# ZhiHuangHn/vtkCloudPoint

Hardware: AMD Instinct MI355X
Metric: Mpoints/s DBSCAN+label @10M pts (higher is better)
Workload: dtype f64; 1 GPU; C4: 10000000-pt cloud (half uniform background, 200 Gaussian blobs), one monolithic DBImproved.dbscan, metric L1_2D, eps 0.1, minPts 10; mode=single, points_total=10000000, points_per_gpu=10000000, clusters=27380, resident_in_hbm=True

## Files before the change

vtkcloudpoint_amd/csrc/dbscan.hip:

```cpp
#include <string.h>

#include <cmath>
#include <cstdlib>
#include <cstring>
#include <limits>
#include <vector>

#include "bounds.hpp"
#include "dbscan_engine.hpp"
#include "grid_common.hpp"

using namespace vcpg;

namespace {

#ifndef VCP_UNR2
#define VCP_UNR2 4
#endif
#ifndef VCP_UNR3
#define VCP_UNR3 2
#endif
#ifndef VCP_UNRW
#define VCP_UNRW 4
#endif
// ... 613 lines not shown
                                                   WorkList wlE, const float* __restrict__ sorted32, Screen sc) {
  const uint32_t p = wl_fetch(wlE);
  if (p == NONE) return;
  float qf[3];
  int cc[3];
  load_pt32<GD>(sorted32, p, qf);
  cell_of32<GD>(qf, g, cc);
  constexpr int UNR = GD == 3 ? VCP_UNR3 : VCP_UNR2;
  const int32_t myg = GROUPED ? sgroup[p] : 0;
  const uint32_t me = (uint32_t)p;
  uint32_t first = me;
  for_rows<GD>(cc, g, ct, [&](uint32_t s, uint32_t e) {
    if (s >= me) return true;
    if (e > me) e = me;
    for (uint32_t j0 = s; j0 < e; j0 += UNR) {
      float rr[UNR][3];
      bool cand[UNR];
#pragma unroll
      for (int u = 0; u < UNR; u++) {
        const uint32_t jj = min(j0 + u, e - 1);
        cand[u] = (j0 + u < e) && (flags[jj] & F_EXPAND);
        if (GROUPED) cand[u] = cand[u] && sgroup[jj] == myg;
        load_pt32<GD>(sorted32, jj, rr[u]);
      }
#pragma unroll
      for (int u = 0; u < UNR; u++)
        if (first == me && cand[u] && within_scr<GD, METRIC>(qf, rr[u], sc, xs, me, j0 + u, thr)) first = j0 + u;
      if (first != me) return false;
    }
    return true;
  });
  if (first != me) parent[me] = first;
}

__global__ __launch_bounds__(TPB) void k_union_init_list(const uint8_t* __restrict__ flags, uint32_t* __restrict__ parent,
                                                        NbrOut no, WorkList wlE) {
  const uint32_t p = wl_fetch(wlE);
  if (p == NONE) return;
  const int nrec = flags[p] >> 4;
  const uint32_t* li = nbr_list(no, p);
  for (int k = 0; k < nrec; k++) {
    const uint32_t j = li[k];
    if (j < p && (flags[j] & F_EXPAND)) {
      parent[p] = j;
      return;
    }
  }
}

template <int JOIN>
__global__ __launch_bounds__(TPB) void k_flatten0(uint32_t* __restrict__ parent, WorkList wlE,
                                                 const uint8_t* __restrict__ flags, NbrOut no) {
  const uint32_t p = wl_fetch(wlE);
  if (p == NONE) return;
  uint32_t r = (uint32_t)p, x = ld_parent_cached(parent, r);
  if (x == r || JOIN == 2) {
    if (!JOIN) return;
    uint32_t rp = JOIN == 2 ? uf_root(parent, p) : p;
    const int nrec = flags[p] >> 4;
    const uint32_t* li = nbr_list(no, p);
    uint32_t s0 = NONE, s1 = NONE, s2 = NONE;
    for (int k = 0; k < nrec; k++) {
      const uint32_t j = li[k];
      if (!(flags[j] & F_EXPAND)) continue;
      const uint32_t y = ld_parent_cached(parent, j);
      if (y == rp || y == s0 || y == s1 || y == s2) continue;
      const uint32_t ry = uf_root(parent, y);
      const uint32_t rm = uf_root(parent, rp);
      s2 = s1;
      s1 = s0;
      s0 = rp;
      rp = (ry != rm) ? uf_link(parent, rm, ry) : rm;
      if (y != rp) s1 = y;
    }
    return;
  }
  while (x != r) {
    r = x;
    x = ld_parent_cached(parent, r);
  }
  __hip_atomic_store(&parent[p], r, __ATOMIC_RELAXED, __HIP_MEMORY_SCOPE_WAVEFRONT);
}

constexpr uint32_t CHUNK_MIXED = 0xFFFFFFFEu;
constexpr int DENSE_PER_CELL = 16;
__global__ __launch_bounds__(TPB) void k_chunkroot(const uint32_t* __restrict__ parent, CellTab ct,
                                                  uint32_t* __restrict__ chunkroot) {
  const uint32_t nin = *ct.nin;
  const int64_t p = (int64_t)blockIdx.x * TPB + threadIdx.x;
  const uint32_t x = p < nin ? parent[p] : NONE;
  const unsigned long long have = __ballot(x != NONE);
  uint32_t out = NONE;
  if (have) {
    const uint32_t r = (uint32_t)__shfl((int)x, __ffsll((long long)have) - 1, 64);
    out = __ballot(x != NONE && x != r) ? CHUNK_MIXED : r;
  }
  if ((threadIdx.x & 63) == 0) chunkroot[p >> 6] = out;
}

#define VCP_JOIN(x)                                                \
  do {                                                             \
    const uint32_t rx__ = uf_root(parent, (x));                    \
    const uint32_t rm__ = uf_root(parent, rp);                     \
    rp = (rx__ != rm__) ? uf_link(parent, rm__, rx__) : rm__;      \
  } while (0)
#define VCP_FLUSH()                                                \
  do {                                                             \
    if (q0 != NONE) {                                              \
      const uint32_t old__ = rp;                                   \
      VCP_JOIN(q0);                                                \
      a2 = a0;                                                     \
      a0 = q0;                                                     \
      a1 = old__;                                                  \
    }                                                              \
    if (q1 != NONE) {                                              \
      VCP_JOIN(q1);                                                \
      a2 = q1;                                                     \
    }                                                              \
    q0 = q1 = NONE;                                                \
  } while (0)

template <int GD, int METRIC, bool GROUPED, bool PRE, bool DENSE = false>
__global__ __launch_bounds__(TPB) void k_union(ExactSrc xs, GridP g, double thr,
                                              CellTab ct,
                                              const int32_t* __restrict__ sgroup, uint32_t* __restrict__ parent,
                                              WorkList wlE, const float* __restrict__ sorted32, Screen sc,
                                              const uint32_t* __restrict__ chunkroot = nullptr) {
  const uint32_t p = wl_fetch(wlE);
  if (p == NONE) return;
  constexpr int NR = GD == 3 ? 9 : 3;
  uint32_t rs[NR], re[NR];
  float qf[3];
  int cc[3];
  load_pt32<GD>(sorted32, p, qf);
  cell_of32<GD>(qf, g, cc);
  row_bounds<GD>(cc, g, ct, rs, re);
  constexpr int UNR = PRE ? VCP_UNRW : (GD == 3 ? VCP_UNR3 : VCP_UNR2);
  const int32_t myg = GROUPED ? sgroup[p] : 0;
  const uint32_t me = (uint32_t)p;
  uint32_t rp = parent[me];
  uint32_t q0 = NONE, q1 = NONE, a0 = NONE, a1 = NONE, a2 = NONE;
#pragma unroll
  for (int r = 0; r < NR; r++) {
    const uint32_t s = rs[r];
    const uint32_t e = min(re[r], me);
    uint32_t last_c = NONE;
    for (uint32_t j0 = s; j0 < e; j0 += UNR) {
      if (DENSE) {
        const uint32_t cj = j0 >> 6;
        if (cj != last_c) {
          last_c = cj;
          if ((cj << 6) >= s && ((cj + 1u) << 6) <= e) {
            const uint32_t cr = chunkroot[cj];
            if (cr == NONE || cr == rp) {
              j0 = ((cj + 1u) << 6) - UNR;
              continue;
            }
          }
        }
      }
      uint32_t pj[UNR];
      float cf[UNR][3];
#pragma unroll
      for (int u = 0; u < UNR; u++) {
        const uint32_t jj = min(j0 + u, e - 1);
        pj[u] = ld_parent_cached(parent, jj);
        if (!PRE) load_pt32<GD>(sorted32, jj, cf[u]);
      }
#pragma unroll
      for (int u = 0; u < UNR; u++) {
        const uint32_t j = j0 + u, x = pj[u];
        if (j >= e || x == NONE || x == rp) continue;
        if (PRE && (x == a0 || x == a1 || x == a2 || x == q0 || x == q1)) continue;
        if (GROUPED && sgroup[j] != myg) continue;
        if (PRE) load_pt32<GD>(sorted32, j, cf[u]);
        if (!within_scr<GD, METRIC>(qf, cf[u], sc, xs, me, j, thr)) continue;
        if (!PRE) {
          const uint32_t x2 = ld_parent_cached(parent, x);
          if (x2 != rp) {
            const uint32_t rx = uf_root(parent, x2);
            const uint32_t rm = uf_root(parent, rp);
            rp = (rx != rm) ? uf_link(parent, rm, rx) : rm;
          }
          if (x != rp && j != rp) __hip_atomic_store(&parent[j], rp, __ATOMIC_RELAXED, __HIP_MEMORY_SCOPE_WAVEFRONT);
        } else if (q0 == NONE) {
          q0 = x;
        } else if (q1 == NONE) {
          q1 = x;
        } else {
          VCP_FLUSH();
          q0 = x;
        }
      }
    }
  }
  VCP_FLUSH();
  if (rp != me) __hip_atomic_store(&parent[me], rp, __ATOMIC_RELAXED, __HIP_MEMORY_SCOPE_AGENT);
}
#undef VCP_FLUSH
#undef VCP_JOIN

template <bool FILTER>
__global__ __launch_bounds__(TPB) void k_flatten(uint32_t* __restrict__ parent, const uint32_t* __restrict__ sord,
                                                uint32_t* __restrict__ minord, WorkList wlE) {
  const uint32_t p = wl_fetch(wlE);
  uint32_t r = NONE, v = NONE;
  if (p != NONE) {
    r = (uint32_t)p;
    uint32_t x = parent[r];
    while (x != r) {
      r = x;
      x = parent[r];
    }
    parent[p] = r;
    v = sord[p];
  }
  unsigned long long todo = __ballot(r != NONE);
  const int lane = threadIdx.x & 63;
  while (todo) {
    int leader = __ffsll((long long)todo) - 1;
    uint32_t lr = __shfl(r, leader, 64);
    bool mine = (r == lr);
    uint32_t m = mine ? v : NONE;
#pragma unroll
    for (int d = 32; d > 0; d >>= 1) m = min(m, (uint32_t)__shfl_xor((int)m, d, 64));
    if (lane == leader &&
        (!FILTER || m < __hip_atomic_load(&minord[lr], __ATOMIC_RELAXED, __HIP_MEMORY_SCOPE_AGENT)))
      atomicMin(&minord[lr], m);
    todo &= ~__ballot(mine);
  }
}

__device__ __forceinline__ uint32_t seed_rank(const uint32_t* __restrict__ bits, const uint32_t* __restrict__ pref,
                                              uint32_t m) {
  const uint32_t w = m >> 5;
  return pref[w] + (uint32_t)__popc(bits[w] & ((1u << (m & 31u)) - 1u));
}
__global__ __launch_bounds__(TPB) void k_seed_popc(const uint32_t* __restrict__ bits, uint32_t nw, uint32_t* __restrict__ cnt) {
  uint32_t w = blockIdx.x * TPB + threadIdx.x;
  if (w < nw) cnt[w] = (uint32_t)__popc(bits[w]);
}

__global__ __launch_bounds__(TPB) void k_seedflag(const uint32_t* __restrict__ parent, const uint32_t* __restrict__ minord,
                                                 uint32_t* __restrict__ seedflag, WorkList wlE) {
  const uint32_t p = wl_fetch(wlE);
  if (p == NONE) return;
  if (parent[p] == p) {
    const uint32_t m = minord[p];
    atomicOr(&seedflag[m >> 5], 1u << (m & 31u));
  }
}

__global__ __launch_bounds__(TPB) void k_rootk(const uint32_t* __restrict__ parent, const uint32_t* __restrict__ minord,
                                              const uint32_t* __restrict__ seedbits, const uint32_t* __restrict__ seedpref,
                                              uint32_t* __restrict__ rootk, uint32_t* __restrict__ clseed, WorkList wlE) {
  const uint32_t p = wl_fetch(wlE);
  if (p == NONE) return;
  if (parent[p] == p) {
    uint32_t k = seed_rank(seedbits, seedpref, minord[p]);
    rootk[p] = k;
    clseed[k] = minord[p];
  }
}

__device__ __forceinline__ void twice_add(unsigned twice, unsigned long long* __restrict__ counters) {
  __shared__ unsigned tw[TPB / 64];
  const unsigned long long m2 = __ballot(twice);
  if ((threadIdx.x & 63) == 0) tw[threadIdx.x >> 6] = (unsigned)__popcll(m2);
  __syncthreads();
  if (threadIdx.x == 0) {
    unsigned t = 0;
    for (int k = 0; k < TPB / 64; k++) t += tw[k];
    if (t) atomicAdd(&counters[CNT_TWICE + (blockIdx.x & (CNT_SPREAD - 1))], (unsigned long long)t);
  }
}

template <int GD, int METRIC, bool GROUPED>
__global__ __launch_bounds__(TPB) void k_border(ExactSrc xs, GridP g, double thr,
                                               CellTab ct,
                                               const int32_t* __restrict__ sgroup, const uint8_t* __restrict__ flags,
                                               const uint32_t* __restrict__ parent, const uint32_t* __restrict__ sord,
                                               const uint32_t* __restrict__ rootk, const uint32_t* __restrict__ clseed,
                                               uint32_t* __restrict__ labk, unsigned long long* __restrict__ counters,
                                               uint32_t* __restrict__ group_twice, WorkList wlB, uint32_t own_lo,
                                               uint32_t own_span, const float* __restrict__ sorted32, Screen sc) {
  const uint32_t p = wl_fetch(wlB);
  unsigned twice = 0;
  if (p != NONE) {
    const uint8_t fl = flags[p];
    uint32_t out = 0;
    {
      float qf[3];
      int cc[3];
      load_pt32<GD>(sorted32, p, qf);
      cell_of32<GD>(qf, g, cc);
      constexpr int UNR = VCP_UNRW;
      const int32_t myg = GROUPED ? sgroup[p] : 0;
      uint32_t mx = 0, mnk = NONE;
      for_rows<GD>(cc, g, ct, [&](uint32_t s, uint32_t e) {
        for (uint32_t j0 = s; j0 < e; j0 += UNR) {
          uint32_t rk[UNR];
#pragma unroll
          for (int u = 0; u < UNR; u++) rk[u] = rootk[min(j0 + u, e - 1)];
#pragma unroll
          for (int u = 0; u < UNR; u++) {
            const uint32_t j = j0 + u, x = rk[u];
            if (j >= e || x == NONE || (x >= mnk && x < mx)) continue;
            if (GROUPED && sgroup[j] != myg) continue;
            float rr[3];
            load_pt32<GD>(sorted32, j, rr);
            if (within_scr<GD, METRIC>(qf, rr, sc, xs, p, j, thr)) {
              mx = max(mx, x + 1u);
              mnk = min(mnk, x);
            }
          }
        }
        return true;
      });
      out = mx;
      if (mx != 0 && !(fl & F_CLASSED) && sord[p] - own_lo < own_span && sord[p] < clseed[mnk]) {
        twice = 1;
        if (GROUPED) atomicAdd(&group_twice[myg], 1u);
      }
    }
    labk[p] = (out << 2) | ((fl & F_CORE) ? 1u : 0u) | ((fl & F_CLASSED) ? 2u : 0u);
  }
  if (!GROUPED) twice_add(twice, counters);
}

template <bool GROUPED>
__global__ __launch_bounds__(TPB) void k_border_list(const int32_t* __restrict__ sgroup, const uint8_t* __restrict__ flags,
                                                    const uint32_t* __restrict__ sord, const uint32_t* __restrict__ rootk,
                                                    const uint32_t* __restrict__ clseed, uint32_t* __restrict__ labk,
                                                    unsigned long long* __restrict__ counters,
                                                    uint32_t* __restrict__ group_twice, NbrOut no, WorkList wlB) {
  const uint32_t p = wl_fetch(wlB);
  unsigned twice = 0;
  if (p != NONE) {
    const uint8_t fl = flags[p];
    const int nrec = fl >> 4;
    uint32_t mx = 0, mnk = NONE;
    const uint32_t* li = nbr_list(no, p);
    for (int k = 0; k < nrec; k++) {
      const uint32_t x = rootk[li[k]];
      if (x == NONE) continue;
// ... 213 lines not shown
  int64_t p = (int64_t)blockIdx.x * TPB + threadIdx.x;
  if (p >= nin) return;
  if ((flags[p] & F_EXPAND) && parent[p] == (uint32_t)p) {
    const uint32_t key = minord[p];
    uint32_t lo = 0, hi = nmap;
    while (lo < hi) {
      const uint32_t mid = (lo + hi) >> 1;
      if (map_rep[mid] < key) lo = mid + 1; else hi = mid;
    }
    if (lo < nmap && map_rep[lo] == key) {
      rootk[p] = map_k[lo];
    } else {
      rootk[p] = 0;
      atomicAdd(missing, 1ull);
    }
  }
}

__global__ __launch_bounds__(TPB) void k_slab_output(int64_t n, const uint32_t* __restrict__ pos,
                                                    const uint32_t* __restrict__ labk, const int32_t* __restrict__ tab_gid,
                                                    int32_t* __restrict__ labels, uint8_t* __restrict__ is_classed) {
  int64_t i = (int64_t)blockIdx.x * TPB + threadIdx.x;
  if (i >= n) return;
  const uint32_t k1 = labk[pos[i]] >> 2;
  const int32_t lab = k1 ? tab_gid[k1 - 1] : 0;
  labels[i] = lab;
  if (is_classed) is_classed[i] = lab != 0;
}

double l2_threshold(double eps) {
  if (std::isinf(eps)) return eps;
  double t = eps * eps;
  if (std::isinf(t)) t = std::numeric_limits<double>::max();
  while (std::sqrt(t) > eps) t = std::nextafter(t, 0.0);
  for (;;) {
    double u = std::nextafter(t, std::numeric_limits<double>::infinity());
    if (std::isinf(u) || std::sqrt(u) > eps) break;
    t = u;
  }
  return t;
}

Screen screen_bounds(int metric, int gd, double thr, double E) {
  Screen sc;
  sc.lo = -1.0f;
  sc.hi = INFINITY;
  if (!(thr >= 0.0) || !std::isfinite(E)) return sc;
  if ((thr > 0.0 && thr < 1e-30) || E > 1e18) return sc;
  const double u = 5.9604644775390625e-08;
  const double alpha = 2.0 * u * E * (1.0 + 2.0 * u);
  double err;
  bool lo_ok = true;
  if (metric == VCP_L1_2D) {
    err = 2.0 * alpha * (1.0 + u) + 2.0 * u * (1.0 + u) * thr;
  } else {
    err = 2.0 * alpha * std::sqrt((double)gd * thr) * (1.0 + u) + (double)gd * alpha * alpha + 6.0 * u * (1.0 + u) * thr;
    lo_ok = std::sqrt(thr) > 4.0 * alpha * std::sqrt((double)gd);
  }
  err = err * 1.0625 + 1e-14 * thr + 1e-300;
  const double lo = thr - err, hi = thr + err;
  if (std::isfinite(hi)) {
    float h = (float)hi;
    if ((double)h < hi) h = std::nextafterf(h, INFINITY);
    sc.hi = h;
  }
  if (lo_ok && lo >= 0.0 && std::isfinite(lo)) {
    float l = (float)lo;
    if ((double)l > lo) l = std::nextafterf(l, -INFINITY);
    sc.lo = l;
  } else if (lo_ok && std::isinf(thr) && thr > 0) {
    sc.lo = 3.4028234663852886e38f;
  }
  return sc;
}

unsigned list_perblk(int64_t n) {
  const int64_t band = (n + 8 * LCHUNK - 1) / (8 * LCHUNK) + 1;
  return vcp_blocks(band, TPB);
}

struct Switches {
  int64_t cells_per_point;
  bool screen_off, lists_off, core_global;
  int core_cap, join_all;
};
const Switches& switches() {
  static const Switches sw = [] {
    Switches s;
    const char* e = getenv("VCP_CELL_BUDGET");
    const long v = e ? atol(e) : 32;
    s.cells_per_point = (int64_t)(v < 1 ? 1 : v > 4096 ? 4096 : v);
    s.screen_off = getenv("VCP_NO_SCREEN") != nullptr;
    s.lists_off = getenv("VCP_NO_LISTS") != nullptr;
    s.core_global = getenv("VCP_CORE_GLOBAL") != nullptr;
    s.core_cap = getenv("VCP_CORE_CAP") ? atoi(getenv("VCP_CORE_CAP")) : -1;
    s.join_all = getenv("VCP_JOIN_ALL") ? atoi(getenv("VCP_JOIN_ALL")) : -1;
    return s;
  }();
  return sw;
}

struct EnginePinned {
  double bounds[8];
  uint32_t unclassed;
  uint32_t n_comp;
  unsigned long long counters[CNT_WORDS];
};
static_assert(sizeof(EnginePinned) <= 1024, "the engine's region of vcp_ctx::pinned");
EnginePinned* engine_pinned(vcp_ctx* ctx) { return reinterpret_cast<EnginePinned*>(ctx->pinned); }

struct Call {
  const double* d_coords;
  int64_t n;
  int stride, metric;
  double eps;
  int min_pts;
  int32_t cf_in;
  const uint8_t* d_in_classed;
  int32_t* d_labels;
  uint8_t *d_is_core, *d_is_classed;
  int32_t* cf_out;
  int64_t* dist_evals;
  const DbscanExt* ext;
  int gd = 2;
  unsigned nb = 0;
  const int32_t* d_group = nullptr;
  const uint32_t* d_ord = nullptr;
  uint32_t* d_group_twice = nullptr;
  int G = 0, glo = 0, ghi = 0;
  bool slab = false;
  double* h = nullptr;
  bool all_finite = false;
  double thr = 0.0;
  GridP g;
  Screen sc{-1.0f, INFINITY};
  bool flags_set = false, part_out = false;
  ExactSrc xs{nullptr, nullptr, 0};
  NbrOut no{nullptr, nullptr, 0, 0};
};
void call_derive(Call& c) {
  const DbscanExt* ext = c.ext;
  const bool grouped = ext && ext->d_group;
  c.gd = c.metric == VCP_L2_3D ? 3 : 2;
  c.nb = vcp_blocks(c.n, TPB);
  c.d_group = grouped ? ext->d_group : nullptr;
  c.d_ord = ext ? ext->d_ord : nullptr;
  c.d_group_twice = grouped ? ext->d_group_twice : nullptr;
  c.G = grouped ? ext->G : 0;
  c.glo = grouped ? ext->only_lo : 0;
  c.ghi = grouped ? (ext->only_hi < 0 ? c.G : ext->only_hi) : 0;
  c.slab = ext && ext->slab;
}
BoundsSrc bounds_src(const Call& c) { return BoundsSrc{c.d_coords, c.n, c.gd, c.stride, c.d_group, c.glo, c.ghi}; }

struct MiscView {
  double* d_part;
  double* d_bounds;
  unsigned long long* counters;
  uint32_t* d_total;
};
struct Workspace : MiscView {
  uint4* ctwords;
  uint32_t* ctdense;
  uint32_t* ctcount;
  CellTab ct;
  uint32_t *cellof, *pos, *sord, *parent, *minord, *rootk, *clseed, *labk;
  float* sorted32;
  uint8_t* flags;
  int32_t* sgroup;
  uint32_t nw;
  uint32_t* seedflag;
  uint32_t* seedpref;
  uint32_t *blkE, *blkB;
  WorkList wlE, wlB;
  unsigned nbl;
};

int ws_reserve_misc(vcp_ctx* ctx, int64_t n) {
  return vcp_ensure(ctx, ctx->b_misc, (size_t)(vcp_bounds_parts(n) * 8 + 96) * sizeof(double));
}
MiscView misc_carve(vcp_ctx* ctx, int64_t n) {
  MiscView m;
  m.d_part = ctx->b_misc.as<double>();
  m.d_bounds = m.d_part + (size_t)vcp_bounds_parts(n) * 8;
  m.counters = reinterpret_cast<unsigned long long*>(m.d_bounds + 8);
  m.d_total = reinterpret_cast<uint32_t*>(m.counters + CNT_SEED_TOTAL);
  return m;
}
static_assert((8 + CNT_WORDS) <= 96, "b_misc: bounds and counters behind the partials");

int ws_reserve(vcp_ctx* ctx, int64_t n, unsigned nb, int gd, bool grouped, uint32_t ncells) {
  const size_t ctw = vcp_ct_words(ncells), ctd = vcp_ct_dense_cap(n, ncells);
  VCP_TRY(vcp_ensure(ctx, ctx->b_ctw, ctw * 16 + 64));
  VCP_TRY(vcp_ensure(ctx, ctx->b_ctd, ctd * 128));
  VCP_TRY(vcp_ensure(ctx, ctx->b_cellof, (size_t)n * 4));
  VCP_TRY(vcp_ensure(ctx, ctx->b_pos, (size_t)n * 4));
  VCP_TRY(vcp_ensure(ctx, ctx->b_sorted32, (size_t)n * (gd == 2 ? 2 : 4) * 4));
  VCP_TRY(vcp_ensure(ctx, ctx->b_sidx, (size_t)n * 4));
  VCP_TRY(vcp_ensure(ctx, ctx->b_flags, (size_t)n));
  VCP_TRY(vcp_ensure(ctx, ctx->b_parent, (size_t)n * 4));
  VCP_TRY(vcp_ensure(ctx, ctx->b_minord, (size_t)n * 4));
  const uint32_t nw = (uint32_t)(n / 32 + 2);
  VCP_TRY(vcp_ensure(ctx, ctx->b_seedflag, ((size_t)nw * 2 + 8) * 4));
  VCP_TRY(vcp_ensure(ctx, ctx->b_rootcl, (size_t)n * 4));
  VCP_TRY(vcp_ensure(ctx, ctx->b_clseed, (size_t)n * 4));
  VCP_TRY(vcp_ensure(ctx, ctx->b_labk, (size_t)n * 4));
  if (grouped) VCP_TRY(vcp_ensure(ctx, ctx->b_sgroup, (size_t)n * 4));
  VCP_TRY(vcp_ensure(ctx, ctx->b_wl, ((size_t)n * 2 + (size_t)(nb + 2) * 2) * 4 + 256));
  return VCP_OK;
}
Workspace ws_carve(vcp_ctx* ctx, int64_t n, unsigned nb, bool grouped, uint32_t ncells) {
  Workspace w;
  static_cast<MiscView&>(w) = misc_carve(ctx, n);
  w.ctwords = ctx->b_ctw.as<uint4>();
  w.ctdense = ctx->b_ctd.as<uint32_t>();
  w.ctcount = reinterpret_cast<uint32_t*>(ctx->b_ctw.as<char>() + vcp_ct_words(ncells) * 16);
  w.ct = CellTab{w.ctwords, w.ctdense, w.ctcount + 1};
  w.cellof = ctx->b_cellof.as<uint32_t>();
  w.pos = ctx->b_pos.as<uint32_t>();
  w.sorted32 = ctx->b_sorted32.as<float>();
  w.sord = ctx->b_sidx.as<uint32_t>();
  w.flags = ctx->b_flags.as<uint8_t>();
  w.parent = ctx->b_parent.as<uint32_t>();
  w.minord = ctx->b_minord.as<uint32_t>();
  w.nw = (uint32_t)(n / 32 + 2);
  w.seedflag = ctx->b_seedflag.as<uint32_t>();
  w.seedpref = w.seedflag + ((w.nw + 3) & ~3u);
  w.rootk = ctx->b_rootcl.as<uint32_t>();
  w.clseed = ctx->b_clseed.as<uint32_t>();
  w.labk = ctx->b_labk.as<uint32_t>();
  w.sgroup = grouped ? ctx->b_sgroup.as<int32_t>() : nullptr;
  w.blkE = ctx->b_wl.as<uint32_t>();
  w.blkB = w.blkE + (nb + 2);
  w.wlE.list = w.blkB + (nb + 2);
  w.wlB.list = w.wlE.list + n;
  w.wlE.scan = w.blkE;
  w.wlB.scan = w.blkB;
  w.wlE.nblk = w.wlB.nblk = nb;
  w.wlE.perblk = w.wlB.perblk = list_perblk(n);
  w.nbl = 8u * LCHUNK * w.wlE.perblk;
  return w;
}

struct Totals {
  uint32_t K;
  unsigned long long unclassed;
  unsigned long long twice;
  unsigned long long slot0;
  unsigned long long group_evals;
};
int read_totals(vcp_ctx* ctx, const MiscView& ws, Totals& t) {
  unsigned long long* hc = engine_pinned(ctx)->counters;
  VCP_HIP(ctx, hipMemcpyAsync(hc, ws.counters, CNT_WORDS * sizeof(unsigned long long), hipMemcpyDeviceToHost, ctx->stream));
  VCP_TRY(vcp_phase_finish(ctx));
  VCP_HIP(ctx, hipStreamSynchronize(ctx->stream));
  t.K = *reinterpret_cast<uint32_t*>(hc + CNT_SEED_TOTAL);
  t.slot0 = hc[CNT_LONELY];
  t.group_evals = hc[CNT_GROUP_EVALS];
  t.unclassed = t.twice = 0;
  for (int k = 0; k < CNT_SPREAD; k++) {
    t.unclassed += hc[CNT_UNCLASSED + k];
    t.twice += hc[CNT_TWICE + k];
  }
  return VCP_OK;
}

int stage_bounds(vcp_ctx* ctx, Call& c) {
  vcp_phase(ctx, "bounds");
  VCP_TRY(ws_reserve_misc(ctx, c.n));
  double* h = engine_pinned(ctx)->bounds;
  if (c.ext && c.ext->h_bbox) {
    for (int a = 0; a < 6; a++) h[a] = c.ext->h_bbox[a];
    h[6] = 0.0;
  } else {
    const MiscView m = misc_carve(ctx, c.n);
    VCP_TRY(vcp_bounds(ctx, bounds_src(c), m.d_part, m.d_bounds, h));
  }
  c.h = h;
  c.all_finite = h[6] == 0.0;
  return VCP_OK;
}

int unclassed_ranks(vcp_ctx* ctx, const Call& c, uint32_t* f, uint32_t* d_total) {
  VCP_LAUNCH(ctx, k_unclassed_flag, dim3(c.nb), dim3(TPB), 0, ctx->stream, c.d_in_classed, f, c.n);
  return vcp_exclusive_scan_u32(ctx, f, f, c.n, d_total);
}

template <int GD, int METRIC>
double box_measure(const double* h) {
  const double wx = h[3] - h[0], wy = h[4] - h[1], wz = GD == 3 ? h[5] - h[2] : 0.0;
  return METRIC == VCP_L1_2D ? std::fabs(wx) + std::fabs(wy)
         : METRIC == VCP_L2_2D ? wx * wx + wy * wy : wx * wx + wy * wy + wz * wz;
}

int run_all_pairs(vcp_ctx* ctx, const Call& c) {
  hipStream_t st = ctx->stream;
  const int64_t n = c.n;
  vcp_phase(ctx, "all_pairs");
  VCP_TRY(vcp_ensure(ctx, ctx->b_seedflag, (size_t)(n + 2) * 4));
  uint32_t* f = ctx->b_seedflag.as<uint32_t>();
  uint32_t* d_tot = reinterpret_cast<uint32_t*>(misc_carve(ctx, n).counters);
  unsigned long long unclassed = (unsigned long long)n;
  if (c.d_in_classed) {
    VCP_TRY(unclassed_ranks(ctx, c, f, d_tot));
    uint32_t* hu = &engine_pinned(ctx)->unclassed;
    VCP_HIP(ctx, hipMemcpyAsync(hu, d_tot, 4, hipMemcpyDeviceToHost, st));
    VCP_HIP(ctx, hipStreamSynchronize(st));
    unclassed = hu[0];
  }
  const int core = n >= (int64_t)c.min_pts;
  const int have_seed = unclassed > 0;
  VCP_LAUNCH(ctx, k_all_pairs, dim3(c.nb), dim3(TPB), 0, st, c.d_in_classed, n, core, have_seed, c.cf_in, c.d_labels,
                  c.d_is_core, c.d_is_classed);
  VCP_TRY(vcp_phase_finish(ctx));
  VCP_HIP(ctx, hipStreamSynchronize(st));
  const int made = core && have_seed;
  if (c.cf_out) *c.cf_out = c.cf_in + made;
  if (c.dist_evals) *c.dist_evals = (int64_t)(unclassed + (unsigned long long)made) * n;
  return VCP_OK;
}

int grid_geometry(vcp_ctx* ctx, Call& c, const Switches& sw, double& Emax) {
  const int GD = c.gd;
// ... 58 lines not shown
      if (d > 1048576) d = 1048576;
      g.D[a] = (int)d;
      ncells *= d;
    }
    if (ncells <= budget || std::isinf(cellw)) break;
    cellw *= 1.25;
  }
  if (ncells > budget) return vcp_fail(ctx, VCP_ERR_TOO_LARGE, "grid does not fit the cell budget");
  Emax = 0.0;
  for (int a = 0; a < GD; a++) Emax = std::fmax(Emax, std::fmax(std::fabs(bbox[a] - g.mn[a]), std::fabs(bbox[3 + a] - g.mn[a])));
  if (!std::isfinite(Emax))
    return vcp_fail(ctx, VCP_ERR_UNSUPPORTED, "the cloud's extent overflows binary64 (coordinate - origin is infinite)");
  g.scale = 1.0;
  if (Emax > 1e30 || (Emax > 0.0 && Emax < 1e-20)) g.scale = std::ldexp(1.0, -std::ilogb(Emax));
  g.inv_h = std::isinf(cellw) ? 0.0 : 1.0 / (cellw * g.scale);
  g.ncells = (uint32_t)ncells;
  return VCP_OK;
}

int stage_grid_build(vcp_ctx* ctx, Call& c, const Workspace& ws) {
  GridBuildArgs ga;
  ga.d_coords = c.d_coords;
  ga.n = c.n;
  ga.stride = c.stride;
  ga.gd = c.gd;
  ga.g = c.g;
  ga.d_group = c.d_group;
  ga.glo = c.glo;
  ga.ghi = c.ghi;
  ga.d_ord = c.d_ord;
  ga.d_in_classed = c.d_in_classed;
  ga.ctwords = ws.ctwords;
  ga.ctdense = ws.ctdense;
  ga.ctcount = ws.ctcount;
  ga.sidx = c.d_ord ? ws.cellof : nullptr;
  ga.sorted32 = ws.sorted32;
  ga.sord = ws.sord;
  ga.sgroup = ws.sgroup;
  ga.flags = ws.flags;
  ga.pos = c.part_out ? nullptr : ws.pos;
  VCP_TRY(vcp_grid_build_partition(ctx, ga));
  c.xs = ExactSrc{c.d_coords, c.d_ord ? ws.cellof : ws.sord, c.stride};
  return VCP_OK;
}

template <int GD, int METRIC, bool GROUPED>
int stage_core(vcp_ctx* ctx, Call& c, const Workspace& ws, const Switches& sw) {
  hipStream_t st = ctx->stream;
  const int64_t n = c.n;
  const unsigned nb = c.nb;
  vcp_phase(ctx, "core_count");
  NbrOut& no = c.no;
  if (!sw.lists_off && !c.d_in_classed && !c.slab && c.min_pts >= 2 && c.min_pts <= 16) {
    no.NB = c.min_pts - 1;
    VCP_TRY(vcp_ensure(ctx, ctx->b_nbr, (size_t)no.NB * (size_t)nb * TPB * 4));
    VCP_TRY(vcp_ensure(ctx, ctx->b_nboff, (size_t)nb * TPB * 2));
    no.nbr = ctx->b_nbr.as<uint32_t>();
    no.off = ctx->b_nboff.as<uint16_t>();
    no.core_cap = (GD == 2 && (uint64_t)n < (uint64_t)c.g.ncells) ? std::min(no.NB, CORE_LIST) : no.NB;
    if (sw.core_cap >= 0) no.core_cap = std::min(no.NB, sw.core_cap);
  }
  const size_t lds_nb = (size_t)no.NB * TPB * 4;
  bool tiled = false;
  if constexpr (GD == 2) {
    if (!GROUPED || !sw.core_global) {
      VCP_LAUNCH(ctx, (k_core_lds<GD, METRIC, GROUPED>), dim3(nb), dim3(TPB), 0, st, c.xs, c.g, c.thr, c.min_pts, ws.ct,
                      ws.sgroup, ws.flags, ws.parent, ws.minord, ws.blkE, ws.blkB, no, ws.sorted32, c.sc, c.flags_set);
      tiled = true;
    }
  }
  if (!tiled)
    VCP_LAUNCH(ctx, (k_core<GD, METRIC, GROUPED>), dim3(nb), dim3(TPB), 2 * lds_nb, st, c.xs, c.g, c.thr, c.min_pts, ws.ct,
                    ws.sgroup, ws.flags, ws.parent, ws.minord, ws.blkE, ws.blkB, no, ws.sorted32, c.sc, c.flags_set);
  VCP_TRY(vcp_exclusive_scan_u32(ctx, ws.blkE, ws.blkE, 2 * ((int64_t)nb + 2), nullptr));
  VCP_LAUNCH(ctx, k_wl_fill, dim3(nb), dim3(TPB), 0, st, ws.flags, ws.ct, ws.blkE, ws.blkB, ws.wlE.list, ws.wlB.list,
                  ws.seedflag, ws.nw, ws.counters, c.d_group_twice, (uint32_t)(GROUPED ? c.G : 0));
  return VCP_OK;
}

template <int GD, int METRIC, bool GROUPED>
int stage_union(vcp_ctx* ctx, const Call& c, const Workspace& ws, const Switches& sw) {
  hipStream_t st = ctx->stream;
  const int64_t n = c.n;
  const unsigned nb = c.nb, nbl = ws.nbl;
  const GridP& g = c.g;
  const NbrOut& no = c.no;
  vcp_phase(ctx, "union");
  const bool pre = GD == 2 || no.NB > 0;
  if (no.NB > 0) {
    VCP_LAUNCH(ctx, k_union_init_list, dim3(nbl), dim3(TPB), 0, st, ws.flags, ws.parent, no, ws.wlE);
    const bool all = sw.join_all >= 0 ? sw.join_all != 0 : (uint64_t)n >= (uint64_t)g.ncells;
    if (all) VCP_LAUNCH(ctx, k_flatten0<2>, dim3(nbl), dim3(TPB), 0, st, ws.parent, ws.wlE, ws.flags, no);
    else VCP_LAUNCH(ctx, k_flatten0<1>, dim3(nbl), dim3(TPB), 0, st, ws.parent, ws.wlE, ws.flags, no);
    VCP_LAUNCH(ctx, k_flatten0<0>, dim3(nbl), dim3(TPB), 0, st, ws.parent, ws.wlE, ws.flags, no);
  } else if (GD == 2) {
    VCP_LAUNCH(ctx, (k_union_init<GD, METRIC, GROUPED>), dim3(nbl), dim3(TPB), 0, st, c.xs, g, c.thr, ws.ct, ws.sgroup,
                    ws.flags, ws.parent, ws.wlE, ws.sorted32, c.sc);
    VCP_LAUNCH(ctx, k_flatten0<0>, dim3(nbl), dim3(TPB), 0, st, ws.parent, ws.wlE, ws.flags, no);
  }
  const bool dense = pre && (uint64_t)n > (uint64_t)DENSE_PER_CELL * g.ncells;
  if (dense) {
    VCP_TRY(vcp_ensure(ctx, ctx->b_aux0, ((size_t)nb * (TPB / 64) + 2) * 4));
    uint32_t* chunkroot = ctx->b_aux0.as<uint32_t>();
    VCP_LAUNCH(ctx, k_chunkroot, dim3(nb), dim3(TPB), 0, st, ws.parent, ws.ct, chunkroot);
    VCP_LAUNCH(ctx, (k_union<GD, METRIC, GROUPED, true, true>), dim3(nbl), dim3(TPB), 0, st, c.xs, g, c.thr, ws.ct,
                    ws.sgroup, ws.parent, ws.wlE, ws.sorted32, c.sc, chunkroot);
  } else if (pre)
    VCP_LAUNCH(ctx, (k_union<GD, METRIC, GROUPED, true>), dim3(nbl), dim3(TPB), 0, st, c.xs, g, c.thr, ws.ct, ws.sgroup,
                    ws.parent, ws.wlE, ws.sorted32, c.sc);
  else
    VCP_LAUNCH(ctx, (k_union<GD, METRIC, GROUPED, false>), dim3(nbl), dim3(TPB), 0, st, c.xs, g, c.thr, ws.ct, ws.sgroup,
                    ws.parent, ws.wlE, ws.sorted32, c.sc);
  return VCP_OK;
}

int stage_slab_handoff(vcp_ctx* ctx, const Call& c, const Workspace& ws) {
  hipStream_t st = ctx->stream;
  const unsigned nb = c.nb;
  vcp_phase(ctx, "slab_components");
  VCP_LAUNCH(ctx, k_slab_count, dim3(nb), dim3(TPB), 0, st, ws.parent, ws.flags, ws.ct, ws.blkE);
  VCP_TRY(vcp_exclusive_scan_u32(ctx, ws.blkE, ws.blkE, (int64_t)nb + 1, nullptr));
  VCP_LAUNCH(ctx, k_slab_fill, dim3(nb), dim3(TPB), 0, st, ws.parent, ws.flags, ws.minord, ws.ct, ws.blkE, ws.clseed);
  VCP_LAUNCH(ctx, k_slab_out, dim3(nb), dim3(TPB), 0, st, c.n, ws.pos, ws.flags, ws.parent, ws.minord, c.ext->d_slab_rep,
                  c.d_is_core);
  uint32_t* hn = &engine_pinned(ctx)->n_comp;
  VCP_HIP(ctx, hipMemcpyAsync(hn, ws.blkE + nb, 4, hipMemcpyDeviceToHost, st));
  VCP_TRY(vcp_phase_finish(ctx));
  VCP_HIP(ctx, hipStreamSynchronize(st));
  if (!ctx->slab) ctx->slab = new SlabState();
  SlabState& ss = *ctx->slab;
  ss.valid = true;
  ss.gd = c.gd;
  ss.metric = c.metric;
  ss.n = c.n;
  ss.n_comp = hn[0];
  ss.g = c.g;
  ss.thr = c.thr;
  ss.sc = c.sc;
  ss.xs = c.xs;
  ss.nb = nb;
  if (c.cf_out) *c.cf_out = (int32_t)hn[0];
  return VCP_OK;
}

template <bool GROUPED>
int stage_flatten_number(vcp_ctx* ctx, const Call& c, const Workspace& ws) {
  hipStream_t st = ctx->stream;
  const unsigned nbl = ws.nbl;
  vcp_phase(ctx, "flatten_number");
  if ((uint64_t)c.n >= (uint64_t)c.g.ncells)
    VCP_LAUNCH(ctx, k_flatten<true>, dim3(nbl), dim3(TPB), 0, st, ws.parent, ws.sord, ws.minord, ws.wlE);
  else
    VCP_LAUNCH(ctx, k_flatten<false>, dim3(nbl), dim3(TPB), 0, st, ws.parent, ws.sord, ws.minord, ws.wlE);
  if (!GROUPED && c.slab) return stage_slab_handoff(ctx, c, ws);
  VCP_LAUNCH(ctx, k_seedflag, dim3(nbl), dim3(TPB), 0, st, ws.parent, ws.minord, ws.seedflag, ws.wlE);
  VCP_LAUNCH(ctx, k_seed_popc, dim3(vcp_blocks(ws.nw, TPB)), dim3(TPB), 0, st, ws.seedflag, ws.nw, ws.seedpref);
  VCP_TRY(vcp_exclusive_scan_u32(ctx, ws.seedpref, ws.seedpref, ws.nw, ws.d_total));
  VCP_LAUNCH(ctx, k_rootk, dim3(nbl), dim3(TPB), 0, st, ws.parent, ws.minord, ws.seedflag, ws.seedpref, ws.rootk, ws.clseed,
                  ws.wlE);
  return VCP_OK;
}

template <int GD, int METRIC, bool GROUPED>
int stage_border(vcp_ctx* ctx, const Call& c, const Workspace& ws) {
  hipStream_t st = ctx->stream;
  vcp_phase(ctx, "border");
  VCP_LAUNCH(ctx, k_labk_rest, dim3(c.nb), dim3(TPB), 0, st, ws.flags, ws.parent, ws.rootk, ws.labk, ws.ct);
  if (c.no.NB > 0)
    VCP_LAUNCH(ctx, k_border_list<GROUPED>, dim3(ws.nbl), dim3(TPB), 0, st, ws.sgroup, ws.flags, ws.sord, ws.rootk,
                    ws.clseed, ws.labk, ws.counters, c.d_group_twice, c.no, ws.wlB);
  else
    VCP_LAUNCH(ctx, (k_border<GD, METRIC, GROUPED>), dim3(ws.nbl), dim3(TPB), 0, st, c.xs, c.g, c.thr, ws.ct, ws.sgroup,
                    ws.flags, ws.parent, ws.sord, ws.rootk, ws.clseed, ws.labk, ws.counters, c.d_group_twice, ws.wlB, 0u,
                    NONE, ws.sorted32, c.sc);
  return VCP_OK;
}

template <int GD, bool GROUPED>
int stage_output(vcp_ctx* ctx, const Call& c, const Workspace& ws) {
  hipStream_t st = ctx->stream;
  const int64_t n = c.n;
  const unsigned nb = c.nb;
  const DbscanExt* ext = c.ext;
  if (c.part_out) {
    GridOutputArgs oa;
    oa.n = n;
    oa.sord = ws.sord;
    oa.labk = ws.labk;
    oa.have_in_classed = c.d_in_classed != nullptr;
    oa.cf_in = c.cf_in;
    oa.labels = c.d_labels;
    oa.is_core = c.d_is_core;
    oa.is_classed = c.d_is_classed;
    oa.counters = ws.counters;
    VCP_TRY(vcp_grid_output_partition(ctx, oa));
  } else {
    vcp_phase(ctx, "output");
    VCP_LAUNCH(ctx, (k_output<GROUPED>), dim3(nb), dim3(TPB), 0, st, n, ws.pos, ws.labk, c.d_in_classed, c.d_group,
                    GROUPED ? ext->d_groupstart : nullptr, ws.seedflag, ws.seedpref, c.cf_in, c.d_labels, c.d_is_core,
                    c.d_is_classed, ws.counters);
  }
  if (!GROUPED && c.min_pts <= 0 && !c.all_finite)
    VCP_LAUNCH(ctx, k_lonely_seeds<GD>, dim3(nb), dim3(TPB), 0, st, c.d_coords, n, c.stride, c.d_in_classed,
                    c.d_is_classed, ws.counters + CNT_LONELY);
  if (GROUPED) {
    VCP_LAUNCH(ctx, k_group_stats, dim3(vcp_blocks(c.G, TPB)), dim3(TPB), 0, st, c.G, c.glo, c.ghi, ext->d_groupstart,
                    ws.seedflag, ws.seedpref, ext->d_group_twice, ext->d_group_nclus, ws.counters + CNT_GROUP_EVALS,
                    ext->skip_upto);
    if (ext->d_group_evals)
      VCP_HIP(ctx, hipMemcpyAsync(ext->d_group_evals, ws.counters + CNT_GROUP_EVALS, 8, hipMemcpyDeviceToDevice, st));
  }
  return VCP_OK;
}

template <int GD, int METRIC, bool GROUPED>
int run_dbscan(vcp_ctx* ctx, Call& c) {
  const Switches& sw = switches();
  VCP_TRY(stage_bounds(ctx, c));
  c.thr = (METRIC == VCP_L1_2D) ? c.eps : l2_threshold(c.eps);
  if (!GROUPED && c.all_finite && !c.slab && box_measure<GD, METRIC>(c.h) <= c.thr) return run_all_pairs(ctx, c);

  double Emax = 0.0;
  VCP_TRY(grid_geometry(ctx, c, sw, Emax));
  c.sc = screen_bounds(METRIC, GD, METRIC == VCP_L1_2D ? c.thr * c.g.scale : c.thr * c.g.scale * c.g.scale, Emax * c.g.scale);
  if (sw.screen_off) c.sc = Screen{-1.0f, INFINITY};

  VCP_TRY(ws_reserve(ctx, c.n, c.nb, GD, GROUPED, c.g.ncells));
  const Workspace ws = ws_carve(ctx, c.n, c.nb, GROUPED, c.g.ncells);
  c.flags_set = c.d_in_classed != nullptr;
  c.part_out = !GROUPED && !c.d_ord && !c.slab && c.n <= ((int64_t)1 << 27);
  VCP_TRY(stage_grid_build(ctx, c, ws));
  VCP_TRY((stage_core<GD, METRIC, GROUPED>(ctx, c, ws, sw)));
  VCP_TRY((stage_union<GD, METRIC, GROUPED>(ctx, c, ws, sw)));
  VCP_TRY(stage_flatten_number<GROUPED>(ctx, c, ws));
  if (!GROUPED && c.slab) return VCP_OK;
  VCP_TRY((stage_border<GD, METRIC, GROUPED>(ctx, c, ws)));
  VCP_TRY((stage_output<GD, GROUPED>(ctx, c, ws)));

  Totals t;
  VCP_TRY(read_totals(ctx, ws, t));
  const unsigned long long unclassed = c.d_in_classed ? t.unclassed : (unsigned long long)c.n;
  if (c.cf_out) *c.cf_out = c.cf_in + (int32_t)t.K;
// ... 250 lines not shown
```

vtkcloudpoint_amd/csrc/grid_common.hpp:

```cpp
#pragma once
#include "vcp_ctx.hpp"

namespace vcpg {

constexpr int TPB = 256;
constexpr uint8_t F_CORE = 1, F_CLASSED = 2, F_EXPAND = 4, F_BCAND = 8;
constexpr uint32_t NONE = 0xFFFFFFFFu;

constexpr int CNT_LONELY = 0, CNT_MISSING = 0, CNT_SEED_TOTAL = 2, CNT_GROUP_EVALS = 3;
constexpr int CNT_SPREAD = 32;
constexpr int CNT_UNCLASSED = 4, CNT_TWICE = CNT_UNCLASSED + CNT_SPREAD, CNT_WORDS = CNT_TWICE + CNT_SPREAD;

struct GridP {
  double mn[3];
  double inv_h;
  double scale;
  int D[3];
  uint32_t ncells;
};

template <int GD>
__device__ __forceinline__ uint32_t cell_id(const GridP& g, int cx, int cy, int cz) {
  uint32_t id = (uint32_t)cy * (uint32_t)g.D[0] + (uint32_t)cx;
  if (GD == 3) id += (uint32_t)cz * (uint32_t)g.D[0] * (uint32_t)g.D[1];
  return id;
}

__device__ __forceinline__ float rel32(double x, double mn, double scale) { return (float)((x - mn) * scale); }

__device__ __forceinline__ int cell_coord32(float f, double inv_h, int D) {
  double u = (double)f * inv_h;
  if (u >= 0.0 && u < (double)D) return (int)u;
  if (u >= (double)D) return D - 1;
  return 0;
}

__device__ __forceinline__ int cell_coord(double x, double mn, double scale, double inv_h, int D) {
  return cell_coord32(rel32(x, mn, scale), inv_h, D);
}

template <int GD>
__device__ __forceinline__ void load_pt(const double* __restrict__ c, int64_t i, double* q) {
  if (GD == 2) {
    double2 v = *reinterpret_cast<const double2*>(c + 2 * i);
    q[0] = v.x;
    q[1] = v.y;
  } else {
    q[0] = c[3 * i];
    q[1] = c[3 * i + 1];
    q[2] = c[3 * i + 2];
  }
}

template <int GD>
__device__ __forceinline__ void store_pt(double* __restrict__ c, int64_t i, const double* q) {
  if (GD == 2) {
    *reinterpret_cast<double2*>(c + 2 * i) = make_double2(q[0], q[1]);
  } else {
    c[3 * i] = q[0];
    c[3 * i + 1] = q[1];
    c[3 * i + 2] = q[2];
  }
}

template <int GD>
__device__ __forceinline__ void load_in(const double* __restrict__ c, int64_t i, int stride, double* q) {
  if (GD == 2 && stride == 2) {
    double2 v = *reinterpret_cast<const double2*>(c + 2 * i);
    q[0] = v.x;
    q[1] = v.y;
  } else {
#pragma unroll
    for (int a = 0; a < GD; a++) q[a] = c[i * stride + a];
  }
}

template <int GD>
__device__ __forceinline__ uint32_t cell_of(const double* q, const GridP& g, int* cc) {
  cc[0] = cell_coord(q[0], g.mn[0], g.scale, g.inv_h, g.D[0]);
  cc[1] = cell_coord(q[1], g.mn[1], g.scale, g.inv_h, g.D[1]);
  cc[2] = 0;
  if (GD == 3) cc[2] = cell_coord(q[2], g.mn[2], g.scale, g.inv_h, g.D[2]);
  return cell_id<GD>(g, cc[0], cc[1], cc[2]);
}

template <int GD>
__device__ __forceinline__ uint32_t cell_of32(const float* qf, const GridP& g, int* cc) {
  cc[0] = cell_coord32(qf[0], g.inv_h, g.D[0]);
  cc[1] = cell_coord32(qf[1], g.inv_h, g.D[1]);
  cc[2] = 0;
  if (GD == 3) cc[2] = cell_coord32(qf[2], g.inv_h, g.D[2]);
  return cell_id<GD>(g, cc[0], cc[1], cc[2]);
}

// ... 102 lines not shown
```

Baseline: 7068 Mpoints/s.

## Compact union-find roots into lists and widen chunk-root skipping in union

```diff
diff --git a/vtkcloudpoint_amd/csrc/dbscan.hip b/vtkcloudpoint_amd/csrc/dbscan.hip
--- a/vtkcloudpoint_amd/csrc/dbscan.hip
+++ b/vtkcloudpoint_amd/csrc/dbscan.hip
@@ -719,20 +719,43 @@
   __hip_atomic_store(&parent[p], r, __ATOMIC_RELAXED, __HIP_MEMORY_SCOPE_WAVEFRONT);
 }
 
+#ifndef VCP_CHUNK_SHIFT
+#define VCP_CHUNK_SHIFT 6
+#endif
 constexpr uint32_t CHUNK_MIXED = 0xFFFFFFFEu;
 constexpr int DENSE_PER_CELL = 16;
+constexpr int CHUNK_SHIFT = VCP_CHUNK_SHIFT, CHUNK = 1 << CHUNK_SHIFT;
+static_assert(CHUNK_SHIFT >= 3 && CHUNK_SHIFT <= 8, "a chunk is shared by 2..64 lanes of one wave");
+inline unsigned chunk_blocks(int64_t n) { return vcp_blocks(n, 4 * TPB); }
+inline size_t chunk_words(int64_t n) { return (size_t)chunk_blocks(n) * (4 * TPB / CHUNK); }
 __global__ __launch_bounds__(TPB) void k_chunkroot(const uint32_t* __restrict__ parent, CellTab ct,
                                                   uint32_t* __restrict__ chunkroot) {
   const uint32_t nin = *ct.nin;
-  const int64_t p = (int64_t)blockIdx.x * TPB + threadIdx.x;
-  const uint32_t x = p < nin ? parent[p] : NONE;
-  const unsigned long long have = __ballot(x != NONE);
-  uint32_t out = NONE;
-  if (have) {
-    const uint32_t r = (uint32_t)__shfl((int)x, __ffsll((long long)have) - 1, 64);
-    out = __ballot(x != NONE && x != r) ? CHUNK_MIXED : r;
-  }
-  if ((threadIdx.x & 63) == 0) chunkroot[p >> 6] = out;
+  const int64_t t = (int64_t)blockIdx.x * TPB + threadIdx.x, p = 4 * t;
+  uint32_t x[4] = {NONE, NONE, NONE, NONE};
+  if (p + 4 <= (int64_t)nin) {
+    const uint4 v = *reinterpret_cast<const uint4*>(parent + p);
+    x[0] = v.x, x[1] = v.y, x[2] = v.z, x[3] = v.w;
+  } else {
+#pragma unroll
+    for (int k = 0; k < 4; k++)
+      if (p + k < (int64_t)nin) x[k] = parent[p + k];
+  }
+  uint32_t mine = NONE;
+  bool mixed = false;
+#pragma unroll
+  for (int k = 0; k < 4; k++) {
+    if (x[k] == NONE) continue;
+    if (mine == NONE) mine = x[k];
+    mixed = mixed || x[k] != mine;
+  }
+  constexpr int GL = CHUNK / 4;
+  const int lane = threadIdx.x & 63, g0 = lane & ~(GL - 1);
+  const unsigned long long gm = (GL == 64 ? ~0ull : ((1ull << GL) - 1ull)) << g0;
+  const unsigned long long have = __ballot(mine != NONE) & gm;
+  const uint32_t r = (uint32_t)__shfl((int)mine, have ? __ffsll((long long)have) - 1 : lane, 64);
+  const unsigned long long bad = __ballot(mixed || (mine != NONE && mine != r)) & gm;
+  if (lane == g0) chunkroot[t / GL] = !have ? NONE : bad ? CHUNK_MIXED : r;
 }
 
 #define VCP_JOIN(x)                                                \
@@ -757,7 +780,7 @@
     q0 = q1 = NONE;                                                \
   } while (0)
 
-template <int GD, int METRIC, bool GROUPED, bool PRE, bool DENSE = false>
+template <int GD, int METRIC, bool GROUPED, bool PRE, bool CHUNKS = false>
 __global__ __launch_bounds__(TPB) void k_union(ExactSrc xs, GridP g, double thr,
                                               CellTab ct,
                                               const int32_t* __restrict__ sgroup, uint32_t* __restrict__ parent,
@@ -783,16 +806,14 @@
     const uint32_t e = min(re[r], me);
     uint32_t last_c = NONE;
     for (uint32_t j0 = s; j0 < e; j0 += UNR) {
-      if (DENSE) {
-        const uint32_t cj = j0 >> 6;
+      if (PRE && CHUNKS) {
+        const uint32_t cj = j0 >> CHUNK_SHIFT;
         if (cj != last_c) {
           last_c = cj;
-          if ((cj << 6) >= s && ((cj + 1u) << 6) <= e) {
-            const uint32_t cr = chunkroot[cj];
-            if (cr == NONE || cr == rp) {
-              j0 = ((cj + 1u) << 6) - UNR;
-              continue;
-            }
+          const uint32_t cr = chunkroot[cj];
+          if (cr == NONE || cr == rp || cr == a0 || cr == a1 || cr == a2) {
+            j0 = ((cj + 1u) << CHUNK_SHIFT) - UNR;
+            continue;
           }
         }
       }
@@ -837,23 +858,53 @@
 #undef VCP_FLUSH
 #undef VCP_JOIN
 
+constexpr unsigned ROOT_GRID = 1024;
+static_assert(ROOT_GRID % CNT_SPREAD == 0, "every segment is walked by the same number of workgroups");
+struct RootList {
+  uint32_t* list;
+  unsigned long long* count;
+  uint32_t cap;
+};
+inline uint32_t root_cap(unsigned nbl) { return (nbl + CNT_SPREAD - 1) / CNT_SPREAD * TPB; }
+template <class F>
+__device__ __forceinline__ void for_roots(const RootList& rl, F&& f) {
+  const uint32_t s = blockIdx.x & (CNT_SPREAD - 1);
+  const uint32_t cnt = min((uint32_t)rl.count[s], rl.cap);
+  const uint32_t* seg = rl.list + (size_t)s * rl.cap;
+  for (uint32_t k = (blockIdx.x / CNT_SPREAD) * TPB + threadIdx.x; k < cnt; k += gridDim.x / CNT_SPREAD * TPB) f(seg[k]);
+}
+
 template <bool FILTER>
 __global__ __launch_bounds__(TPB) void k_flatten(uint32_t* __restrict__ parent, const uint32_t* __restrict__ sord,
-                                                uint32_t* __restrict__ minord, WorkList wlE) {
+                                                uint32_t* __restrict__ minord, WorkList wlE, RootList rl) {
   const uint32_t p = wl_fetch(wlE);
-  uint32_t r = NONE, v = NONE;
+  uint32_t r = NONE, v = NONE, x = NONE;
+  if (p != NONE) {
+    x = parent[p];
+    v = sord[p];
+  }
+  __shared__ unsigned wr[TPB / 64];
+  __shared__ uint32_t wbase;
+  const int lane = threadIdx.x & 63, w = threadIdx.x >> 6;
+  const bool isroot = p != NONE && x == p;
+  const unsigned long long roots = __ballot(isroot);
+  const uint32_t seg = blockIdx.x & (CNT_SPREAD - 1);
+  if (lane == 0) wr[w] = (unsigned)__popcll(roots);
+  __syncthreads();
+  if (threadIdx.x == 0) {
+    unsigned t = 0;
+    for (int k = 0; k < TPB / 64; k++) t += wr[k];
+    wbase = t ? atomicAdd(reinterpret_cast<uint32_t*>(rl.count + seg), t) : 0u;
+  }
   if (p != NONE) {
     r = (uint32_t)p;
-    uint32_t x = parent[r];
     while (x != r) {
       r = x;
       x = parent[r];
     }
     parent[p] = r;
-    v = sord[p];
   }
   unsigned long long todo = __ballot(r != NONE);
-  const int lane = threadIdx.x & 63;
   while (todo) {
     int leader = __ffsll((long long)todo) - 1;
     uint32_t lr = __shfl(r, leader, 64);
@@ -866,6 +917,12 @@
       atomicMin(&minord[lr], m);
     todo &= ~__ballot(mine);
   }
+  __syncthreads();
+  if (isroot) {
+    uint32_t k = wbase + (uint32_t)__popcll(roots & ((1ull << lane) - 1ull));
+    for (int q = 0; q < w; q++) k += wr[q];
+    if (k < rl.cap) rl.list[(size_t)seg * rl.cap + k] = p;
+  }
 }
 
 __device__ __forceinline__ uint32_t seed_rank(const uint32_t* __restrict__ bits, const uint32_t* __restrict__ pref,
@@ -878,26 +935,23 @@
   if (w < nw) cnt[w] = (uint32_t)__popc(bits[w]);
 }
 
-__global__ __launch_bounds__(TPB) void k_seedflag(const uint32_t* __restrict__ parent, const uint32_t* __restrict__ minord,
-                                                 uint32_t* __restrict__ seedflag, WorkList wlE) {
-  const uint32_t p = wl_fetch(wlE);
-  if (p == NONE) return;
-  if (parent[p] == p) {
+__global__ __launch_bounds__(TPB) void k_seedflag(const uint32_t* __restrict__ minord, uint32_t* __restrict__ seedflag,
+                                                 RootList rl) {
+  for_roots(rl, [&](uint32_t p) {
     const uint32_t m = minord[p];
     atomicOr(&seedflag[m >> 5], 1u << (m & 31u));
-  }
-}
-
-__global__ __launch_bounds__(TPB) void k_rootk(const uint32_t* __restrict__ parent, const uint32_t* __restrict__ minord,
-                                              const uint32_t* __restrict__ seedbits, const uint32_t* __restrict__ seedpref,
-                                              uint32_t* __restrict__ rootk, uint32_t* __restrict__ clseed, WorkList wlE) {
-  const uint32_t p = wl_fetch(wlE);
-  if (p == NONE) return;
-  if (parent[p] == p) {
-    uint32_t k = seed_rank(seedbits, seedpref, minord[p]);
+  });
+}
+
+__global__ __launch_bounds__(TPB) void k_rootk(const uint32_t* __restrict__ minord, const uint32_t* __restrict__ seedbits,
+                                              const uint32_t* __restrict__ seedpref, uint32_t* __restrict__ rootk,
+                                              uint32_t* __restrict__ clseed, RootList rl) {
+  for_roots(rl, [&](uint32_t p) {
+    const uint32_t m = minord[p];
+    const uint32_t k = seed_rank(seedbits, seedpref, m);
     rootk[p] = k;
-    clseed[k] = minord[p];
-  }
+    clseed[k] = m;
+  });
 }
 
 __device__ __forceinline__ void twice_add(unsigned twice, unsigned long long* __restrict__ counters) {
@@ -1277,7 +1331,7 @@
 struct Switches {
   int64_t cells_per_point;
   bool screen_off, lists_off, core_global;
-  int core_cap, join_all;
+  int core_cap, join_all, union_chunks;
 };
 const Switches& switches() {
   static const Switches sw = [] {
@@ -1290,6 +1344,7 @@
     s.core_global = getenv("VCP_CORE_GLOBAL") != nullptr;
     s.core_cap = getenv("VCP_CORE_CAP") ? atoi(getenv("VCP_CORE_CAP")) : -1;
     s.join_all = getenv("VCP_JOIN_ALL") ? atoi(getenv("VCP_JOIN_ALL")) : -1;
+    s.union_chunks = getenv("VCP_UNION_CHUNKS") ? atoi(getenv("VCP_UNION_CHUNKS")) : -1;
     return s;
   }();
   return sw;
@@ -1369,10 +1424,11 @@
   uint32_t *blkE, *blkB;
   WorkList wlE, wlB;
   unsigned nbl;
+  RootList roots;
 };
 
 int ws_reserve_misc(vcp_ctx* ctx, int64_t n) {
-  return vcp_ensure(ctx, ctx->b_misc, (size_t)(vcp_bounds_parts(n) * 8 + 96) * sizeof(double));
+  return vcp_ensure(ctx, ctx->b_misc, (size_t)(vcp_bounds_parts(n) * 8 + 128) * sizeof(double));
 }
 MiscView misc_carve(vcp_ctx* ctx, int64_t n) {
   MiscView m;
@@ -1382,7 +1438,7 @@
   m.d_total = reinterpret_cast<uint32_t*>(m.counters + CNT_SEED_TOTAL);
   return m;
 }
-static_assert((8 + CNT_WORDS) <= 96, "b_misc: bounds and counters behind the partials");
+static_assert((8 + CNT_WORDS) <= 128, "b_misc: bounds and counters behind the partials");
 
 int ws_reserve(vcp_ctx* ctx, int64_t n, unsigned nb, int gd, bool grouped, uint32_t ncells) {
   const size_t ctw = vcp_ct_words(ncells), ctd = vcp_ct_dense_cap(n, ncells);
@@ -1399,7 +1455,7 @@
   VCP_TRY(vcp_ensure(ctx, ctx->b_seedflag, ((size_t)nw * 2 + 8) * 4));
   VCP_TRY(vcp_ensure(ctx, ctx->b_rootcl, (size_t)n * 4));
   VCP_TRY(vcp_ensure(ctx, ctx->b_clseed, (size_t)n * 4));
-  VCP_TRY(vcp_ensure(ctx, ctx->b_labk, (size_t)n * 4));
+  VCP_TRY(vcp_ensure(ctx, ctx->b_labk, std::max((size_t)n, (size_t)CNT_SPREAD * root_cap(8u * LCHUNK * list_perblk(n))) * 4));
   if (grouped) VCP_TRY(vcp_ensure(ctx, ctx->b_sgroup, (size_t)n * 4));
   VCP_TRY(vcp_ensure(ctx, ctx->b_wl, ((size_t)n * 2 + (size_t)(nb + 2) * 2) * 4 + 256));
   return VCP_OK;
@@ -1434,6 +1490,7 @@
   w.wlE.nblk = w.wlB.nblk = nb;
   w.wlE.perblk = w.wlB.perblk = list_perblk(n);
   w.nbl = 8u * LCHUNK * w.wlE.perblk;
+  w.roots = RootList{w.labk, w.counters + CNT_ROOTS, root_cap(w.nbl)};
   return w;
 }
 
@@ -1658,7 +1715,7 @@
 int stage_union(vcp_ctx* ctx, const Call& c, const Workspace& ws, const Switches& sw) {
   hipStream_t st = ctx->stream;
   const int64_t n = c.n;
-  const unsigned nb = c.nb, nbl = ws.nbl;
+  const unsigned nbl = ws.nbl;
   const GridP& g = c.g;
   const NbrOut& no = c.no;
   vcp_phase(ctx, "union");
@@ -1674,11 +1731,12 @@
                     ws.flags, ws.parent, ws.wlE, ws.sorted32, c.sc);
     VCP_LAUNCH(ctx, k_flatten0<0>, dim3(nbl), dim3(TPB), 0, st, ws.parent, ws.wlE, ws.flags, no);
   }
-  const bool dense = pre && (uint64_t)n > (uint64_t)DENSE_PER_CELL * g.ncells;
-  if (dense) {
-    VCP_TRY(vcp_ensure(ctx, ctx->b_aux0, ((size_t)nb * (TPB / 64) + 2) * 4));
+  const bool chunks =
+      pre && (sw.union_chunks >= 0 ? sw.union_chunks != 0 : GD == 3 || (uint64_t)n > (uint64_t)DENSE_PER_CELL * g.ncells);
+  if (chunks) {
+    VCP_TRY(vcp_ensure(ctx, ctx->b_aux0, chunk_words(n) * 4));
     uint32_t* chunkroot = ctx->b_aux0.as<uint32_t>();
-    VCP_LAUNCH(ctx, k_chunkroot, dim3(nb), dim3(TPB), 0, st, ws.parent, ws.ct, chunkroot);
+    VCP_LAUNCH(ctx, k_chunkroot, dim3(chunk_blocks(n)), dim3(TPB), 0, st, ws.parent, ws.ct, chunkroot);
     VCP_LAUNCH(ctx, (k_union<GD, METRIC, GROUPED, true, true>), dim3(nbl), dim3(TPB), 0, st, c.xs, g, c.thr, ws.ct,
                     ws.sgroup, ws.parent, ws.wlE, ws.sorted32, c.sc, chunkroot);
   } else if (pre)
@@ -1725,15 +1783,15 @@
   const unsigned nbl = ws.nbl;
   vcp_phase(ctx, "flatten_number");
   if ((uint64_t)c.n >= (uint64_t)c.g.ncells)
-    VCP_LAUNCH(ctx, k_flatten<true>, dim3(nbl), dim3(TPB), 0, st, ws.parent, ws.sord, ws.minord, ws.wlE);
+    VCP_LAUNCH(ctx, k_flatten<true>, dim3(nbl), dim3(TPB), 0, st, ws.parent, ws.sord, ws.minord, ws.wlE, ws.roots);
   else
-    VCP_LAUNCH(ctx, k_flatten<false>, dim3(nbl), dim3(TPB), 0, st, ws.parent, ws.sord, ws.minord, ws.wlE);
+    VCP_LAUNCH(ctx, k_flatten<false>, dim3(nbl), dim3(TPB), 0, st, ws.parent, ws.sord, ws.minord, ws.wlE, ws.roots);
   if (!GROUPED && c.slab) return stage_slab_handoff(ctx, c, ws);
-  VCP_LAUNCH(ctx, k_seedflag, dim3(nbl), dim3(TPB), 0, st, ws.parent, ws.minord, ws.seedflag, ws.wlE);
+  VCP_LAUNCH(ctx, k_seedflag, dim3(ROOT_GRID), dim3(TPB), 0, st, ws.minord, ws.seedflag, ws.roots);
   VCP_LAUNCH(ctx, k_seed_popc, dim3(vcp_blocks(ws.nw, TPB)), dim3(TPB), 0, st, ws.seedflag, ws.nw, ws.seedpref);
   VCP_TRY(vcp_exclusive_scan_u32(ctx, ws.seedpref, ws.seedpref, ws.nw, ws.d_total));
-  VCP_LAUNCH(ctx, k_rootk, dim3(nbl), dim3(TPB), 0, st, ws.parent, ws.minord, ws.seedflag, ws.seedpref, ws.rootk, ws.clseed,
-                  ws.wlE);
+  VCP_LAUNCH(ctx, k_rootk, dim3(ROOT_GRID), dim3(TPB), 0, st, ws.minord, ws.seedflag, ws.seedpref, ws.rootk, ws.clseed,
+                  ws.roots);
   return VCP_OK;
 }
 
diff --git a/vtkcloudpoint_amd/csrc/grid_common.hpp b/vtkcloudpoint_amd/csrc/grid_common.hpp
--- a/vtkcloudpoint_amd/csrc/grid_common.hpp
+++ b/vtkcloudpoint_amd/csrc/grid_common.hpp
@@ -9,7 +9,8 @@
 
 constexpr int CNT_LONELY = 0, CNT_MISSING = 0, CNT_SEED_TOTAL = 2, CNT_GROUP_EVALS = 3;
 constexpr int CNT_SPREAD = 32;
-constexpr int CNT_UNCLASSED = 4, CNT_TWICE = CNT_UNCLASSED + CNT_SPREAD, CNT_WORDS = CNT_TWICE + CNT_SPREAD;
+constexpr int CNT_UNCLASSED = 4, CNT_TWICE = CNT_UNCLASSED + CNT_SPREAD, CNT_ROOTS = CNT_TWICE + CNT_SPREAD,
+              CNT_WORDS = CNT_ROOTS + CNT_SPREAD;
 
 struct GridP {
   double mn[3];
```

New measurement: 7135 Mpoints/s, median of 6. No clear change (+0.9%).
